# openMVG/openMVG

Hardware: AMD Instinct MI355X
Metric: descriptor pairs/s (brute-force L2 2-NN + ratio matching) (higher is better)
Workload: dtype i8 (int32 accumulate); 1 GPU; 1000 images x 2000 SIFT-like uint8x128 descriptors, exhaustive pairs (499500 image pairs, 499500 on rank 0), ratio 0.8; parallelism=pair-sharded x1, no collective

## Files before the change

openmvg_amd/csrc/mvgx_match.hip:

```cpp
#include <hip/hip_runtime.h>

#include <algorithm>
#include <atomic>
#include <climits>
#include <condition_variable>
#include <cstdint>
#include <cstdlib>
#include <cstring>
#include <functional>
#include <mutex>
#include <string>
#include <thread>
#include <vector>

#include "mvgx_common.h"

namespace {

using mvgx::set_error;

typedef int v4i __attribute__((ext_vector_type(4)));
typedef int v16i __attribute__((ext_vector_type(16)));

constexpr int kDim = 128;
// ... 316 lines not shown
    for (int n = 0; n < kNQ; ++n) { T1[n] = INT_MIN; T2[n] = INT_MIN; }

    const int nt = min(kWinTiles, ntI - win * kWinTiles);
    for (int t = 0; t < nt; ++t) {
      const char* tb = buf + t * kTileBytes + lane * 16;
      v4i a[4];
#pragma unroll
      for (int s = 0; s < 4; ++s) a[s] = *reinterpret_cast<const v4i*>(tb + s * 1024);
      const char* rb = buf + kWinTiles * kTileBytes + t * (kTileRows * 4) + h * 16;
      int R[16];
#pragma unroll
      for (int g = 0; g < 4; ++g) {
        const int4 rv = *reinterpret_cast<const int4*>(rb + g * 32);
        R[g * 4 + 0] = rv.x; R[g * 4 + 1] = rv.y; R[g * 4 + 2] = rv.z; R[g * 4 + 3] = rv.w;
      }
#pragma unroll
      for (int n = 0; n < kNQ; ++n) {
        v16i acc = {0, 0, 0, 0, 0, 0, 0, 0, 0, 0, 0, 0, 0, 0, 0, 0};
#pragma unroll
        for (int s = 0; s < 4; ++s) acc = __builtin_amdgcn_mfma_i32_32x32x32_i8(a[s], b[n][s], acc, 0, 0, 0);
        int t1 = T1[n], t2 = T2[n];
#pragma unroll
        for (int r = 0; r < 16; ++r) {
          const int T = (int)((unsigned)acc[r] << 9) + R[r];
          t2 = med3i(t1, t2, T);
          t1 = max(t1, T);
        }
        T1[n] = t1; T2[n] = t2;
      }
    }
    if constexpr (kMode == kStageRegs) stage_commit(nbuf, sr, wave, lane);
#pragma unroll
    for (int n = 0; n < kNQ; ++n) {
      const int k1 = -T1[n], k2 = -T2[n];
      const int wd1 = k1 >> 8, widx = (k1 & 255) + win * kWinRows, wd2 = k2 >> 8;
      const bool better = wd1 < G1[n];
      const int g2 = better ? min(G1[n], wd2) : min(G2[n], wd1);
      Gi[n] = better ? widx : Gi[n];
      G1[n] = better ? wd1 : G1[n];
      G2[n] = g2;
    }
  }

#pragma unroll
  for (int n = 0; n < kNQ; ++n) {
    const int P1 = __shfl_xor(G1[n], 32), P2 = __shfl_xor(G2[n], 32), Pi = __shfl_xor(Gi[n], 32);
    const bool better = P1 < G1[n];
    const int g2 = better ? min(G1[n], P2) : min(G2[n], P1);
    Gi[n] = better ? Pi : Gi[n];
    G1[n] = better ? P1 : G1[n];
    G2[n] = g2;
  }

#pragma unroll
  for (int n = 0; n < kNQ; ++n) {
    const uint32_t q = (qt0 + n) * kTileRows + (lane & 31);
    const bool inb = (lane < 32) && (qt0 + n < ntJpad);
    bool ok = false;
    if (inb) {
      const bool valid = p.perm[(size_t)tileJ0 * kTileRows + q] != kNoMatch;
      const int nq = p.qnorm[(size_t)tileJ0 * kTileRows + q];
      const int d0 = G1[n] + nq, d1 = G2[n] + nq;
      ok = valid && (__int2float_rn(d0) < __fmul_rn(p.ratio_sq, __int2float_rn(d1)));
      p.best[(size_t)wk.x * p.qstride + q] = ok ? p.perm[(size_t)tileI0 * kTileRows + (uint32_t)Gi[n]] : kNoMatch;
    }
    const unsigned long long m = __ballot(ok);
    if (lane == 0 && m) atomicAdd(&p.count[wk.x], (uint32_t)__popcll(m));
  }
}

__device__ __forceinline__ int max3i(int a, int b, int c) { return max(max(a, b), c); }

template <int kMode, int kDbg = 0>
__global__ __launch_bounds__(256, 2) void l2_filter_kernel(MatchParams p) {
  extern __shared__ __attribute__((aligned(16))) char smem[];

  const int lane = threadIdx.x & 63;
  const int wave = __builtin_amdgcn_readfirstlane(threadIdx.x >> 6);
  const int h = lane >> 5;

  const uint32_t w = xcd_remap(blockIdx.x, gridDim.x);
  const uint2 wk = p.work[w];
  const uint2 ij = p.pairs[wk.x];
  const uint32_t I = ij.x, J = ij.y;
  const uint32_t tileI0 = p.img_tile_off[I], tileJ0 = p.img_tile_off[J];
  const uint32_t ntJpad = p.img_tile_off[J + 1] - tileJ0;
  const int ntI = (int)p.img_ntiles[I];
  const int nwin = (ntI + kWinTiles - 1) / kWinTiles;
  const uint32_t qt0 = wk.y + (uint32_t)wave * kNQ;

  v4i b[kNQ][4];
  {
    const int8_t* qsrc = p.tiles + (size_t)(tileJ0 + qt0) * kTileBytes + lane * 16;
#pragma unroll
    for (int n = 0; n < kNQ; ++n)
#pragma unroll
      for (int s = 0; s < 4; ++s) b[n][s] = *reinterpret_cast<const v4i*>(qsrc + n * kTileBytes + s * 1024);
  }

  const int8_t* gI = p.tiles + (size_t)tileI0 * kTileBytes;
  const int* gC = p.cinit + (size_t)tileI0 * kTileRows;

  constexpr bool kFold = (kDbg & 8) == 0;
  constexpr bool kOneCv = kFold && (kDbg & 16) != 0;
  int TP[kNQ][8];
  int TW[kNQ][8];
  int Q1[kNQ], Q2[kNQ], Qg[kNQ];
#pragma unroll
  for (int n = 0; n < kNQ; ++n) {
#pragma unroll
    for (int s = 0; s < 8; ++s) { TP[n][s] = kNegInit; TW[n][s] = kNegInit; }
    Q1[n] = kNegInit; Q2[n] = kNegInit; Qg[n] = 0;
  }

  StageRegs sr;
  if constexpr (kMode == kStageGlds) {
    stage_window_glds(smem, gI, gC, wave, lane);
  } else if constexpr (kMode == kStageGldsAsm) {
    stage_window_glds_asm(smem, gI, gC, wave, lane);
  } else {
    stage_issue(sr, gI, gC, wave, lane);
    stage_commit(smem, sr, wave, lane);
  }
#pragma unroll
  for (int n = 0; n < kNQ; ++n)
#pragma unroll
    for (int s = 0; s < 4; ++s) asm volatile("" : "+v"(b[n][s]));

  for (int win = 0; win < nwin; ++win) {
    if constexpr (!(kDbg & 4) && kMode == kStageGldsAsm) asm volatile("s_waitcnt vmcnt(0)" ::: "memory");
    if constexpr (!(kDbg & 4)) __syncthreads();
    char* buf = smem + (win & 1) * kStageBytes;
    char* nbuf = smem + ((win + 1) & 1) * kStageBytes;
    if constexpr (kDbg & 4) {
    } else if constexpr (kMode == kStageRegs) {
      const int wn = (win + 1 < nwin) ? win + 1 : win;
      stage_issue(sr, gI + (size_t)wn * kWinTiles * kTileBytes, gC + wn * kWinRows, wave, lane);
    } else if (win + 1 < nwin) {
      const int8_t* gt = gI + (size_t)(win + 1) * kWinTiles * kTileBytes;
      const int* gc = gC + (win + 1) * kWinRows;
      if constexpr (kMode == kStageGlds) stage_window_glds(nbuf, gt, gc, wave, lane);
      else stage_window_glds_asm(nbuf, gt, gc, wave, lane);
    }

    int TQ[kNQ];
#pragma unroll
    for (int n = 0; n < kNQ; ++n) TQ[n] = kNegInit;

    const int nt = min(kWinTiles, ntI - win * kWinTiles);
    const char* wb = buf + lane * 16;
    const char* wc = buf + kWinTiles * kTileBytes + h * 16;
    v4i a[4];
    v16i cv;
#pragma unroll
    for (int s = 0; s < 4; ++s) a[s] = *reinterpret_cast<const v4i*>(wb + s * 1024);
#pragma unroll
    for (int g = 0; g < 4; ++g) {
      const int4 c4 = *reinterpret_cast<const int4*>(wc + g * 32);
      cv[g * 4 + 0] = c4.x; cv[g * 4 + 1] = c4.y; cv[g * 4 + 2] = c4.z; cv[g * 4 + 3] = c4.w;
    }
    v16i accA, accB;
#pragma unroll
    for (int r = 0; r < 16; ++r) accB[r] = kNegInit;

#define MVGX_EPILOGUE(ACC, N)                                          \
  if constexpr (kDbg & 1) { asm volatile("" : "+v"(ACC)); TQ[N] = max(TQ[N], ACC[0]); } else \
  if constexpr (kFold) {                                               \
    _Pragma("unroll") for (int s = 0; s < 8; ++s)                      \
      TW[N][s] = max(max(TW[N][s], ACC[2 * s]), ACC[2 * s + 1]);       \
  } else                                                               \
  {                                                                    \
    int tq = TQ[N];                                                    \
    _Pragma("unroll") for (int s = 0; s < 8; ++s) {                    \
      TP[N][s] = max(max(TP[N][s], ACC[2 * s]), ACC[2 * s + 1]);       \
      tq = max(max(tq, ACC[2 * s + 1]), ACC[2 * s]);                   \
    }                                                                  \
    TQ[N] = tq;                                                        \
  }
#define MVGX_CHAIN(ACC, N, A, CV)                                                            \
  ACC = __builtin_amdgcn_mfma_i32_32x32x32_i8(A[0], b[N][0], CV, 0, 0, 0);                   \
  ACC = __builtin_amdgcn_mfma_i32_32x32x32_i8(A[1], b[N][1], ACC, 0, 0, 0);                  \
  ACC = __builtin_amdgcn_mfma_i32_32x32x32_i8(A[2], b[N][2], ACC, 0, 0, 0);                  \
  ACC = __builtin_amdgcn_mfma_i32_32x32x32_i8(A[3], b[N][3], ACC, 0, 0, 0);
#define MVGX_INTERLEAVE()                                                                    \
  _Pragma("unroll") for (int i_ = 0; i_ < 4; ++i_) {                                         \
    __builtin_amdgcn_sched_group_barrier(0x8, 1, 0);                                         \
    __builtin_amdgcn_sched_group_barrier(0x2, kFold ? 2 : 4, 0);                             \
  }

#define MVGX_TILE(A, CV, AN, CN, TN)                                                              \
  {                                                                                                \
    const int tn_ = (TN);                                                                          \
    MVGX_CHAIN(accA, 0, A, CV)                                                                     \
    if constexpr (kDbg & 2) { _Pragma("unroll") for (int s = 0; s < 4; ++s) AN[s] = A[s]; CN = CV; } else { \
    _Pragma("unroll") for (int s = 0; s < 4; ++s)                                                  \
        AN[s] = *reinterpret_cast<const v4i*>(wb + tn_ * kTileBytes + s * 1024);                   \
    }                                                                                              \
    MVGX_EPILOGUE(accB, 3)                                                                         \
    MVGX_INTERLEAVE()                                                                              \
    MVGX_CHAIN(accB, 1, A, CV)                                                                     \
    if constexpr (!(kDbg & 2) && !kOneCv) {                                                        \
    _Pragma("unroll") for (int g = 0; g < 4; ++g) {                                                \
      const int4 c4 = *reinterpret_cast<const int4*>(wc + tn_ * (kTileRows * 4) + g * 32);        \
      CN[g * 4 + 0] = c4.x; CN[g * 4 + 1] = c4.y; CN[g * 4 + 2] = c4.z; CN[g * 4 + 3] = c4.w;     \
    }                                                                                              \
    }                                                                                              \
    MVGX_EPILOGUE(accA, 0)                                                                         \
    MVGX_INTERLEAVE()                                                                              \
    MVGX_CHAIN(accA, 2, A, CV)                                                                     \
    MVGX_EPILOGUE(accB, 1)                                                                         \
    MVGX_INTERLEAVE()                                                                              \
    if constexpr (kOneCv) {   \
      accB = __builtin_amdgcn_mfma_i32_32x32x32_i8(A[0], b[3][0], CV, 0, 0, 0);                   \
      if constexpr (!(kDbg & 2))                                                                   \
      _Pragma("unroll") for (int g = 0; g < 4; ++g) {                                              \
        const int4 c4 = *reinterpret_cast<const int4*>(wc + tn_ * (kTileRows * 4) + g * 32);      \
        CV[g * 4 + 0] = c4.x; CV[g * 4 + 1] = c4.y; CV[g * 4 + 2] = c4.z; CV[g * 4 + 3] = c4.w;   \
      }                                                                                            \
      accB = __builtin_amdgcn_mfma_i32_32x32x32_i8(A[1], b[3][1], accB, 0, 0, 0);                 \
      accB = __builtin_amdgcn_mfma_i32_32x32x32_i8(A[2], b[3][2], accB, 0, 0, 0);                 \
      accB = __builtin_amdgcn_mfma_i32_32x32x32_i8(A[3], b[3][3], accB, 0, 0, 0);                 \
    } else {                                                                                       \
      MVGX_CHAIN(accB, 3, A, CV)                                                                   \
    }                                                                                              \
    MVGX_EPILOGUE(accA, 2)                                                                         \
    MVGX_INTERLEAVE()                                                                              \
  }
    v4i an[4];
    v16i cn;
    int t = 0;
    if constexpr (kOneCv) {
      for (; t + 1 < nt; t += 2) {
        MVGX_TILE(a, cv, an, cv, t + 1)
        MVGX_TILE(an, cv, a, cv, min(t + 2, nt - 1))
      }
      if (t < nt) MVGX_TILE(a, cv, an, cv, t)
    } else {
      for (; t + 1 < nt; t += 2) {
        MVGX_TILE(a, cv, an, cn, t + 1)
        MVGX_TILE(an, cn, a, cv, min(t + 2, nt - 1))
      }
      if (t < nt) MVGX_TILE(a, cv, an, cn, t)
    }
    MVGX_EPILOGUE(accB, 3)
#undef MVGX_EPILOGUE
#undef MVGX_CHAIN
#undef MVGX_TILE
#undef MVGX_INTERLEAVE
    if constexpr (kMode == kStageRegs) stage_commit(nbuf, sr, wave, lane);
    if constexpr (kFold) {
#pragma unroll
      for (int n = 0; n < kNQ; ++n) {
        int tq = max(max(TW[n][0], TW[n][1]), TW[n][2]);
        tq = max(max(tq, TW[n][3]), TW[n][4]);
        tq = max(max(tq, TW[n][5]), TW[n][6]);
        TQ[n] = max(tq, TW[n][7]);
#pragma unroll
        for (int s = 0; s < 8; ++s) { TP[n][s] = max(TP[n][s], TW[n][s]); TW[n][s] = kNegInit; }
      }
    }
#pragma unroll
    for (int n = 0; n < kNQ; ++n) {
      const int v = TQ[n];
      const bool better = v > Q1[n];
      Q2[n] = better ? Q1[n] : max(Q2[n], v);
      Qg[n] = better ? win : Qg[n];
      Q1[n] = better ? v : Q1[n];
    }
  }

#pragma unroll
  for (int n = 0; n < kNQ; ++n) {
    int p1 = kNegInit, p2 = kNegInit, ps = 0;
#pragma unroll
    for (int s = 0; s < 8; ++s) {
      const int v = TP[n][s];
      const bool better = v > p1;
      p2 = better ? p1 : max(p2, v);
      ps = better ? s : ps;
      p1 = better ? v : p1;
    }
    const int w1 = 2 * p1 - h, w2p = 2 * p2 - h, w2q = 2 * Q2[n] - h;
    const int o1 = __shfl_xor(w1, 32), o2p = __shfl_xor(w2p, 32), o2q = __shfl_xor(w2q, 32);
    const int os = __shfl_xor(ps, 32), og = __shfl_xor(Qg[n], 32);
    const bool mine = w1 > o1;
    const int W1 = mine ? w1 : o1;
    const int V2 = mine ? max3i(w2p, w2q, o1) : max3i(o2p, o2q, w1);
    const int s1 = mine ? ps : os, g1 = mine ? Qg[n] : og, hw = mine ? h : (h ^ 1);

    const uint32_t q = (qt0 + n) * kTileRows + (lane & 31);
    if (lane < 32 && qt0 + n < ntJpad) {
      const bool valid = p.perm[(size_t)tileJ0 * kTileRows + q] != kNoMatch;
      const int nq = p.qnorm[(size_t)tileJ0 * kTileRows + q];
      const int d0 = nq - W1, d1ub = nq - V2;
      const bool cand = valid && (__int2float_rn(d0) < __fmul_rn(p.ratio_sq, __int2float_rn(d1ub)));
      const size_t o = (size_t)wk.x * p.qstride + q;
      p.best[o] = cand ? ((uint32_t)s1 | ((uint32_t)hw << 3) | ((uint32_t)g1 << 4)) : kNoMatch;
      if (cand) p.cd[o] = make_int2(d0, d1ub);
    }
  }
}

constexpr int kNB16 = 2 * kNQ;
__global__ __launch_bounds__(256, 2) void l2_filter16_kernel(MatchParams p) {
  extern __shared__ __attribute__((aligned(16))) char smem[];

  const int lane = threadIdx.x & 63;
  const int wave = __builtin_amdgcn_readfirstlane(threadIdx.x >> 6);
  const int g4 = lane >> 4, par = g4 & 1;

  const uint32_t w = xcd_remap(blockIdx.x, gridDim.x);
  const uint4* rec = p.work8 + (size_t)kRecQuads * w;
  const uint4 wsh = rec[0], wun = rec[1 + wave];
  const uint32_t tileI0 = wsh.x;
  const int ntI = (int)wsh.y;
  const uint32_t pair = wun.x, tileJ0 = wun.y, qt0 = wun.z;
  const uint32_t nJ = wun.w;
  const int nwin = (ntI + kWinTiles - 1) / kWinTiles;

  const int lane_chunk = ((lane >> 5) * 64 + ((lane >> 4) & 1) * 32 + (lane & 15)) * 16;
  v4i b[kNB16][2];
  {
    const int8_t* qsrc = p.qtiles + (size_t)(tileJ0 + qt0) * kTileBytes + lane_chunk;
#pragma unroll
    for (int n = 0; n < kNB16; ++n)
#pragma unroll
      for (int ks = 0; ks < 2; ++ks) b[n][ks] = *reinterpret_cast<const v4i*>(qsrc + (n >> 1) * kTileBytes + (n & 1) * 256 + ks * 2048);
  }

  const int8_t* gI = p.tiles + (size_t)tileI0 * kTileBytes;
  const int* gC = p.cinit + (size_t)tileI0 * kTileRows;

  int qn[kNB16];
#pragma unroll
  for (int n = 0; n < kNB16; ++n) {
    const uint32_t q = (qt0 + (uint32_t)(n >> 1)) * kTileRows + (uint32_t)(n & 1) * 16 + (uint32_t)(lane & 15);
    qn[n] = (lane < 16 && q < nJ) ? p.qtnorm[(size_t)tileJ0 * kTileRows + q] : 0;
  }

  int TP[kNB16][4];
  int TW[kNB16][4];
  int Q1[kNB16], Q2[kNB16], Qg[kNB16];
#pragma unroll
  for (int n = 0; n < kNB16; ++n) {
#pragma unroll
    for (int c = 0; c < 4; ++c) { TP[n][c] = kNegInit; TW[n][c] = kNegInit; }
    Q1[n] = kNegInit; Q2[n] = kNegInit; Qg[n] = 0;
  }

  stage_window_glds_asm(smem, gI, gC, wave, lane);
#pragma unroll
  for (int n = 0; n < kNB16; ++n) {
#pragma unroll
    for (int ks = 0; ks < 2; ++ks) asm volatile("" : "+v"(b[n][ks]));
    asm volatile("" : "+v"(qn[n]));
  }

  for (int win = 0; win < nwin; ++win) {
    asm volatile("s_waitcnt vmcnt(0)" ::: "memory");
    __syncthreads();
    char* buf = smem + (win & 1) * kStageBytes;
    char* nbuf = smem + ((win + 1) & 1) * kStageBytes;
    if (win + 1 < nwin)
      stage_window_glds_asm(nbuf, gI + (size_t)(win + 1) * kWinTiles * kTileBytes, gC + (win + 1) * kWinRows, wave, lane);

    const int nt = min(kWinTiles, ntI - win * kWinTiles);
    const char* wb = buf + lane_chunk;
    const char* wc = buf + kWinTiles * kTileBytes + g4 * 16;
    v4i accA[4], accB[4];
#pragma unroll
    for (int i = 0; i < 4; ++i) accB[i] = v4i{kNegInit, kNegInit, kNegInit, kNegInit};

#define MVGX_GROUP16(ACC, N0, A, CV)                                                                       \
  _Pragma("unroll") for (int i_ = 0; i_ < 4; ++i_)                                                          \
    ACC[i_] = __builtin_amdgcn_mfma_i32_16x16x64_i8(A[0], b[(N0) + i_][0], CV, 0, 0, 0);                    \
  _Pragma("unroll") for (int i_ = 0; i_ < 4; ++i_)                                                          \
    ACC[i_] = __builtin_amdgcn_mfma_i32_16x16x64_i8(A[1], b[(N0) + i_][1], ACC[i_], 0, 0, 0);
#define MVGX_EPI16(ACC, N0, BLK)                                                                            \
  _Pragma("unroll") for (int i_ = 0; i_ < 4; ++i_) {                                                        \
    TW[(N0) + i_][2 * (BLK)] = max(max(TW[(N0) + i_][2 * (BLK)], ACC[i_][0]), ACC[i_][1]);                  \
    TW[(N0) + i_][2 * (BLK) + 1] = max(max(TW[(N0) + i_][2 * (BLK) + 1], ACC[i_][2]), ACC[i_][3]);          \
  }
#define MVGX_MIX16(NDS)                                                                                     \
  _Pragma("unroll") for (int i_ = 0; i_ < 8; ++i_) {                                                        \
    __builtin_amdgcn_sched_group_barrier(0x8, 1, 0);                                                        \
    __builtin_amdgcn_sched_group_barrier(0x2, 1, 0);                                                        \
    if (i_ < (NDS)) __builtin_amdgcn_sched_group_barrier(0x100, 1, 0);                                      \
  }
#define MVGX_BLOCK16(A, CV, AN, CN, BLK, NEXT_OFF, NEXT_COFF)                                               \
  {                                                                                                         \
    MVGX_GROUP16(accA, 0, A, CV)                                                                            \
    AN[0] = *reinterpret_cast<const v4i*>(wb + (NEXT_OFF));                                                 \
    AN[1] = *reinterpret_cast<const v4i*>(wb + (NEXT_OFF) + 2048);                                          \
    MVGX_EPI16(accB, 4, 1 - (BLK))                                                                          \
    MVGX_MIX16(2)                                                                                           \
    MVGX_GROUP16(accB, 4, A, CV)                                                                            \
    CN = *reinterpret_cast<const v4i*>(wc + (NEXT_COFF));                                                   \
    MVGX_EPI16(accA, 0, BLK)                                                                                \
    MVGX_MIX16(1)                                                                                           \
  }
    v4i a0[2], a1[2], c0, c1;
    a0[0] = *reinterpret_cast<const v4i*>(wb);
    a0[1] = *reinterpret_cast<const v4i*>(wb + 2048);
    c0 = *reinterpret_cast<const v4i*>(wc);
    __builtin_amdgcn_s_setprio(3);
    for (int t = 0; t < nt; ++t) {
      const int tn = min(t + 1, nt - 1);
      MVGX_BLOCK16(a0, c0, a1, c1, 0, t * kTileBytes + 256, t * (kTileRows * 4) + 64)
      MVGX_BLOCK16(a1, c1, a0, c0, 1, tn * kTileBytes, tn * (kTileRows * 4))
    }
    MVGX_EPI16(accB, 4, 1)
    __builtin_amdgcn_s_setprio(0);
#undef MVGX_GROUP16
#undef MVGX_EPI16
#undef MVGX_MIX16
#undef MVGX_BLOCK16
#pragma unroll
    for (int n = 0; n < kNB16; ++n) {
      const int v = max(max(max(TW[n][0], TW[n][1]), TW[n][2]), TW[n][3]);
#pragma unroll
      for (int c = 0; c < 4; ++c) { TP[n][c] = max(TP[n][c], TW[n][c]); TW[n][c] = kNegInit; }
      const bool better = v > Q1[n];
      Q2[n] = better ? Q1[n] : max(Q2[n], v);
      Qg[n] = better ? win : Qg[n];
      Q1[n] = better ? v : Q1[n];
    }
  }

#pragma unroll
  for (int n = 0; n < kNB16; ++n) {
    int p1 = kNegInit, p2 = kNegInit, pc = 0;
#pragma unroll
    for (int c = 0; c < 4; ++c) {
      const int v = TP[n][c];
      const bool better = v > p1;
      p2 = better ? p1 : max(p2, v);
      pc = better ? c : pc;
      p1 = better ? v : p1;
    }
    int W1 = 2 * p1 - par, V2 = max(2 * p2 - par, 2 * Q2[n] - par);
    int code = (4 * (pc >> 1) + 2 * (g4 >> 1) + (pc & 1)) | (par << 3) | (Qg[n] << 4);
#pragma unroll
    for (int x = 16; x <= 32; x <<= 1) {
      const int o1 = __shfl_xor(W1, x), o2 = __shfl_xor(V2, x), oc = __shfl_xor(code, x);
      const bool mine = W1 > o1;
      V2 = mine ? max(V2, o1) : max(o2, W1);
      code = mine ? code : oc;
      W1 = mine ? W1 : o1;
    }
    const uint32_t q = (qt0 + (uint32_t)(n >> 1)) * kTileRows + (uint32_t)(n & 1) * 16 + (uint32_t)(lane & 15);
    if (lane < 16 && q < nJ) {
      const int nq = qn[n];
      const int d0 = nq - W1, d1ub = nq - V2;
      const bool cand = __int2float_rn(d0) < __fmul_rn(p.ratio_sq, __int2float_rn(d1ub));
      const size_t o = (size_t)pair * p.qstride + q;
      p.best[o] = cand ? (uint32_t)code : kNoMatch;
      if (cand) p.cd[o] = make_int2(d0, d1ub);
    }
  }
}

constexpr int kNQh = 2;
constexpr int kNBh = 2 * kNQh;
constexpr int kBlockQTilesH = kWaves * kNQh;
__global__ __launch_bounds__(256, 3) void l2_filter16h_kernel(MatchParams p) {
  extern __shared__ __attribute__((aligned(16))) char smem[];

  const int lane = threadIdx.x & 63;
  const int wave = __builtin_amdgcn_readfirstlane(threadIdx.x >> 6);
  const int g4 = lane >> 4, par = g4 & 1;

  const uint32_t w = xcd_remap(blockIdx.x, gridDim.x);
  const uint4 wr0 = p.work8h[2 * (size_t)w], wr1 = p.work8h[2 * (size_t)w + 1];
  const uint32_t pair = wr0.x;
  const uint32_t tileI0 = wr0.z, tileJ0 = wr0.w;
  const uint32_t ntJpad = wr1.y;
  const int ntI = (int)wr1.x;
  const int nhalf = (ntI + kHalfTiles - 1) / kHalfTiles;
  const uint32_t qt0 = wr0.y + (uint32_t)wave * kNQh;

  const int lane_chunk = ((lane >> 5) * 64 + ((lane >> 4) & 1) * 32 + (lane & 15)) * 16;
  v4i b[kNBh][2];
  {
    const int8_t* qsrc = p.tiles + (size_t)(tileJ0 + qt0) * kTileBytes + lane_chunk;
#pragma unroll
    for (int n = 0; n < kNBh; ++n)
#pragma unroll
      for (int ks = 0; ks < 2; ++ks) b[n][ks] = *reinterpret_cast<const v4i*>(qsrc + (n >> 1) * kTileBytes + (n & 1) * 256 + ks * 2048);
  }
  const int8_t* gI = p.tiles + (size_t)tileI0 * kTileBytes;
  const int* gC = p.cinit + (size_t)tileI0 * kTileRows;

  uint32_t qperm[kNBh];
  int qn[kNBh];
#pragma unroll
  for (int n = 0; n < kNBh; ++n) {
    const bool inb = lane < 16 && qt0 + (uint32_t)(n >> 1) < ntJpad;
    const size_t qs = (size_t)tileJ0 * kTileRows + (qt0 + (uint32_t)(n >> 1)) * kTileRows + (uint32_t)(n & 1) * 16 + (uint32_t)(lane & 15);
    qperm[n] = inb ? p.perm[qs] : kNoMatch;
    qn[n] = inb ? p.qnorm[qs] : 0;
  }

  int TP[kNBh][4], TW[kNBh][4], Q1[kNBh], Q2[kNBh], Qg[kNBh];
#pragma unroll
  for (int n = 0; n < kNBh; ++n) {
#pragma unroll
    for (int c = 0; c < 4; ++c) { TP[n][c] = kNegInit; TW[n][c] = kNegInit; }
    Q1[n] = kNegInit; Q2[n] = kNegInit; Qg[n] = 0;
  }

  stage_half_glds_asm(smem, gI, gC, wave, lane);
#pragma unroll
  for (int n = 0; n < kNBh; ++n) {
#pragma unroll
    for (int ks = 0; ks < 2; ++ks) asm volatile("" : "+v"(b[n][ks]));
    asm volatile("" : "+v"(qperm[n]), "+v"(qn[n]));
  }

  for (int hw = 0; hw < nhalf; ++hw) {
    asm volatile("s_waitcnt vmcnt(0)" ::: "memory");
    __syncthreads();
    char* buf = smem + (hw & 1) * kHalfStageBytes;
    char* nbuf = smem + ((hw + 1) & 1) * kHalfStageBytes;
    if (hw + 1 < nhalf)
      stage_half_glds_asm(nbuf, gI + (size_t)(hw + 1) * kHalfTiles * kTileBytes, gC + (hw + 1) * kHalfTiles * kTileRows, wave, lane);

    const int nt = min(kHalfTiles, ntI - hw * kHalfTiles);
    const char* wb = buf + lane_chunk;
    const char* wc = buf + kHalfTiles * kTileBytes + g4 * 16;
    v4i accA[4], accB[4];
#pragma unroll
    for (int i = 0; i < 4; ++i) accB[i] = v4i{kNegInit, kNegInit, kNegInit, kNegInit};
#define MVGX_GROUPH(ACC, A, CV)                                                                              \
  _Pragma("unroll") for (int i_ = 0; i_ < 4; ++i_)                                                          \
    ACC[i_] = __builtin_amdgcn_mfma_i32_16x16x64_i8(A[0], b[i_][0], CV, 0, 0, 0);                           \
  _Pragma("unroll") for (int i_ = 0; i_ < 4; ++i_)                                                          \
    ACC[i_] = __builtin_amdgcn_mfma_i32_16x16x64_i8(A[1], b[i_][1], ACC[i_], 0, 0, 0);
#define MVGX_EPIH(ACC, BLK)                                                                                  \
  _Pragma("unroll") for (int i_ = 0; i_ < 4; ++i_) {                                                        \
    TW[i_][2 * (BLK)] = max(max(TW[i_][2 * (BLK)], ACC[i_][0]), ACC[i_][1]);                                \
    TW[i_][2 * (BLK) + 1] = max(max(TW[i_][2 * (BLK) + 1], ACC[i_][2]), ACC[i_][3]);                        \
  }
#define MVGX_MIXH(NDS)                                                                                       \
  _Pragma("unroll") for (int i_ = 0; i_ < 8; ++i_) {                                                        \
    __builtin_amdgcn_sched_group_barrier(0x8, 1, 0);                                                        \
    __builtin_amdgcn_sched_group_barrier(0x2, 1, 0);                                                        \
    if (i_ < (NDS)) __builtin_amdgcn_sched_group_barrier(0x100, 1, 0);                                      \
  }
    v4i a0[2], a1[2], c0, c1;
    a0[0] = *reinterpret_cast<const v4i*>(wb);
    a0[1] = *reinterpret_cast<const v4i*>(wb + 2048);
    c0 = *reinterpret_cast<const v4i*>(wc);
    for (int t = 0; t < nt; ++t) {
      const int tn = min(t + 1, nt - 1);
      MVGX_GROUPH(accA, a0, c0)
      a1[0] = *reinterpret_cast<const v4i*>(wb + t * kTileBytes + 256);
      a1[1] = *reinterpret_cast<const v4i*>(wb + t * kTileBytes + 256 + 2048);
      c1 = *reinterpret_cast<const v4i*>(wc + t * (kTileRows * 4) + 64);
      MVGX_EPIH(accB, 1)
      MVGX_MIXH(3)
      MVGX_GROUPH(accB, a1, c1)
      a0[0] = *reinterpret_cast<const v4i*>(wb + tn * kTileBytes);
      a0[1] = *reinterpret_cast<const v4i*>(wb + tn * kTileBytes + 2048);
      c0 = *reinterpret_cast<const v4i*>(wc + tn * (kTileRows * 4));
      MVGX_EPIH(accA, 0)
      MVGX_MIXH(3)
    }
    MVGX_EPIH(accB, 1)
#undef MVGX_GROUPH
#undef MVGX_EPIH
#undef MVGX_MIXH
    if ((hw & 1) || hw + 1 == nhalf) {
      const int win = hw >> 1;
#pragma unroll
      for (int n = 0; n < kNBh; ++n) {
        const int v = max(max(max(TW[n][0], TW[n][1]), TW[n][2]), TW[n][3]);
#pragma unroll
        for (int c = 0; c < 4; ++c) { TP[n][c] = max(TP[n][c], TW[n][c]); TW[n][c] = kNegInit; }
        const bool better = v > Q1[n];
        Q2[n] = better ? Q1[n] : max(Q2[n], v);
        Qg[n] = better ? win : Qg[n];
        Q1[n] = better ? v : Q1[n];
      }
    }
  }

#pragma unroll
  for (int n = 0; n < kNBh; ++n) {
    int p1 = kNegInit, p2 = kNegInit, pc = 0;
#pragma unroll
    for (int c = 0; c < 4; ++c) {
      const int v = TP[n][c];
      const bool better = v > p1;
      p2 = better ? p1 : max(p2, v);
      pc = better ? c : pc;
      p1 = better ? v : p1;
    }
    int W1 = 2 * p1 - par, V2 = max(2 * p2 - par, 2 * Q2[n] - par);
    int code = (4 * (pc >> 1) + 2 * (g4 >> 1) + (pc & 1)) | (par << 3) | (Qg[n] << 4);
#pragma unroll
    for (int x = 16; x <= 32; x <<= 1) {
      const int o1 = __shfl_xor(W1, x), o2 = __shfl_xor(V2, x), oc = __shfl_xor(code, x);
      const bool mine = W1 > o1;
      V2 = mine ? max(V2, o1) : max(o2, W1);
      code = mine ? code : oc;
      W1 = mine ? W1 : o1;
    }
    const uint32_t q = (qt0 + (uint32_t)(n >> 1)) * kTileRows + (uint32_t)(n & 1) * 16 + (uint32_t)(lane & 15);
    if (lane < 16 && qt0 + (uint32_t)(n >> 1) < ntJpad) {
      const bool valid = qperm[n] != kNoMatch;
      const int nq = qn[n];
      const int d0 = nq - W1, d1ub = nq - V2;
      const bool cand = valid && (__int2float_rn(d0) < __fmul_rn(p.ratio_sq, __int2float_rn(d1ub)));
      const size_t o = (size_t)pair * p.qstride + q;
      p.best[o] = cand ? (uint32_t)code : kNoMatch;
      if (cand) p.cd[o] = make_int2(d0, d1ub);
    }
  }
}

template <bool kWaveUnits>
__global__ __launch_bounds__(256) void l2_verify_kernel(MatchParams p) {
  const int lane = threadIdx.x & 63;
  const int wave = threadIdx.x >> 6;
  uint32_t pair, qt0, I, tileI0, tileJ0, qend;
  const uint8_t* rowsJ = nullptr;
  if constexpr (kWaveUnits) {
    const uint4* rec = p.work8 + (size_t)kRecQuads * blockIdx.x;
    const uint4 wun = rec[1 + __builtin_amdgcn_readfirstlane(wave)];
    pair = wun.x; tileJ0 = wun.y; qt0 = wun.z; qend = wun.w;
    tileI0 = rec[0].x;
    const uint2 ij = p.pairs[pair];
    I = ij.x;
    rowsJ = p.rows_u8 + p.img_row_off[ij.y] * kDim;
  } else {
    const uint2 wk = p.work[blockIdx.x];
    const uint2 ij = p.pairs[wk.x];
    pair = wk.x; qt0 = wk.y + (uint32_t)wave * kNQ;
    I = ij.x;
    tileI0 = p.img_tile_off[I]; tileJ0 = p.img_tile_off[ij.y];
    qend = (p.img_tile_off[ij.y + 1] - tileJ0) * kTileRows;
  }
  const uint32_t nEvenI = p.img_neven[I], nOddI = p.img_n[I] - nEvenI;
  const int l16 = lane & 15, sub = lane >> 4;
  uint32_t accepted = 0;
  for (int part = 0; part < 2; ++part) {
    const uint32_t q0 = qt0 * kTileRows + (uint32_t)part * 64;
    const uint32_t q = q0 + lane;
    const bool inb = q < qend;
    const uint32_t code = inb ? p.best[(size_t)pair * p.qstride + q] : kNoMatch;
    unsigned long long todo = __ballot(code != kNoMatch);
    while (todo) {
      unsigned long long m = todo;
      for (int i = 0; i < sub; ++i) m &= m - 1;
      const bool active = m != 0;
      const int src = active ? __builtin_ctzll(m) : 0;
      for (int i = 0; i < 4; ++i) todo &= todo - 1;
      const uint32_t cc = (uint32_t)__shfl((int)code, src);
      const uint32_t qs = q0 + (uint32_t)src;
      const int s1 = cc & 7, hw = (cc >> 3) & 1, g1 = (int)(cc >> 4);
      const int piece = l16 & 7, rsel = l16 >> 3;
      const int mrow = slot_row(2 * s1 + rsel, hw);
      const size_t slot0 = (size_t)tileI0 * kTileRows + (active ? (size_t)g1 * kWinTiles * kTileRows + mrow : 0);
      const size_t slotQ = (size_t)tileJ0 * kTileRows + (active ? qs : 0);
      const size_t o = (size_t)pair * p.qstride + (active ? qs : 0);
      const uint32_t tt = (uint32_t)g1 * kWinTiles + (uint32_t)piece;
      const size_t slotI = active ? slot0 + (size_t)piece * kTileRows : slot0;
      const bool valid = active && (tt * 16u + (uint32_t)(2 * s1 + rsel)) < (hw ? nOddI : nEvenI);
      int4 va[8];
#pragma unroll
      for (int c = 0; c < 8; ++c)
        va[c] = *reinterpret_cast<const int4*>(p.rows_slot + (slot0 + (active ? (size_t)c * kTileRows : 0)) * kDim + piece * 16);
      int4 vb;
      if constexpr (kWaveUnits) {
        vb = *reinterpret_cast<const int4*>(rowsJ + (size_t)(active ? qs : 0) * kDim + piece * 16);
        vb.x ^= (int)0x80808080u; vb.y ^= (int)0x80808080u; vb.z ^= (int)0x80808080u; vb.w ^= (int)0x80808080u;
      } else {
        vb = *reinterpret_cast<const int4*>(p.rows_slot + slotQ * kDim + piece * 16);
      }
      const int2 f = p.cd[o];
      const int f_d0 = f.x, f_d1 = f.y;
      int nb = __builtin_amdgcn_sdot4(vb.x, vb.x, 0, false);
      nb = __builtin_amdgcn_sdot4(vb.y, vb.y, nb, false);
      nb = __builtin_amdgcn_sdot4(vb.z, vb.z, nb, false);
      nb = __builtin_amdgcn_sdot4(vb.w, vb.w, nb, false);
      nb += __builtin_amdgcn_update_dpp(0, nb, 0xB1, 0xF, 0xF, true);
      nb += __builtin_amdgcn_update_dpp(0, nb, 0x4E, 0xF, 0xF, true);
      nb += __builtin_amdgcn_update_dpp(0, nb, 0x141, 0xF, 0xF, true);
      int dot = 0, na = 0;
#pragma unroll
      for (int c = 0; c < 8; ++c) {
        int part = __builtin_amdgcn_sdot4(va[c].x, vb.x, 0, false);
        part = __builtin_amdgcn_sdot4(va[c].y, vb.y, part, false);
        part = __builtin_amdgcn_sdot4(va[c].z, vb.z, part, false);
        part = __builtin_amdgcn_sdot4(va[c].w, vb.w, part, false);
        part += __builtin_amdgcn_update_dpp(0, part, 0xB1, 0xF, 0xF, true);
        part += __builtin_amdgcn_update_dpp(0, part, 0x4E, 0xF, 0xF, true);
        part += __builtin_amdgcn_update_dpp(0, part, 0x141, 0xF, 0xF, true);
        dot = (c == piece) ? part : dot;
        int sq = __builtin_amdgcn_sdot4(va[c].x, va[c].x, 0, false);
        sq = __builtin_amdgcn_sdot4(va[c].y, va[c].y, sq, false);
        sq = __builtin_amdgcn_sdot4(va[c].z, va[c].z, sq, false);
        sq = __builtin_amdgcn_sdot4(va[c].w, va[c].w, sq, false);
        sq += __builtin_amdgcn_update_dpp(0, sq, 0xB1, 0xF, 0xF, true);
        sq += __builtin_amdgcn_update_dpp(0, sq, 0x4E, 0xF, 0xF, true);
        sq += __builtin_amdgcn_update_dpp(0, sq, 0x141, 0xF, 0xF, true);
        na = (c == piece) ? sq : na;
      }
      const int d = valid ? na + nb - 2 * dot : INT_MAX;
      int key = valid ? ((d << 4) | l16) : INT_MAX;
      key = min(key, __builtin_amdgcn_update_dpp(INT_MAX, key, 0xB1, 0xF, 0xF, false));
      key = min(key, __builtin_amdgcn_update_dpp(INT_MAX, key, 0x4E, 0xF, 0xF, false));
      key = min(key, __builtin_amdgcn_update_dpp(INT_MAX, key, 0x141, 0xF, 0xF, false));
      key = min(key, __builtin_amdgcn_update_dpp(INT_MAX, key, 0x140, 0xF, 0xF, false));
      const int wl = key & 15, dbest = key >> 4;
      int second = (l16 == wl) ? INT_MAX : d;
      second = min(second, __builtin_amdgcn_update_dpp(INT_MAX, second, 0xB1, 0xF, 0xF, false));
      second = min(second, __builtin_amdgcn_update_dpp(INT_MAX, second, 0x4E, 0xF, 0xF, false));
      second = min(second, __builtin_amdgcn_update_dpp(INT_MAX, second, 0x141, 0xF, 0xF, false));
      second = min(second, __builtin_amdgcn_update_dpp(INT_MAX, second, 0x140, 0xF, 0xF, false));
      bool ok = false;
      if (active && l16 == wl) {
        if (key == INT_MAX || dbest != f_d0) atomicAdd(p.errflag, 1u);
        const int d1 = min(f_d1, second);
        ok = __int2float_rn(dbest) < __fmul_rn(p.ratio_sq, __int2float_rn(d1));
        p.best[o] = ok ? p.perm[slotI] : kNoMatch;
      }
      accepted += (uint32_t)__popcll(__ballot(ok));
    }
  }
  if (lane == 0 && accepted) atomicAdd(&p.count[pair], accepted);
}

__global__ __launch_bounds__(256) void count_candidates_kernel(const uint32_t* __restrict__ best, size_t n,
                                                               uint32_t* __restrict__ counter) {
  __shared__ uint32_t s_sum;
  if (threadIdx.x == 0) s_sum = 0;
  __syncthreads();
  uint32_t c = 0;
  const size_t base = (size_t)blockIdx.x * 16384;
  for (int k = 0; k < 64; ++k) {
    const size_t i = base + (size_t)k * 256 + threadIdx.x;
    if (i < n && best[i] != kNoMatch) ++c;
  }
  const unsigned long long m = __ballot(c != 0);
  (void)m;
  for (int off = 32; off > 0; off >>= 1) c += __shfl_down(c, off);
  if ((threadIdx.x & 63) == 0 && c) atomicAdd(&s_sum, c);
  __syncthreads();
  if (threadIdx.x == 0 && s_sum) atomicAdd(counter, s_sum);
}

__global__ __launch_bounds__(256) void count_candidates_units_kernel(MatchParams p, uint32_t* __restrict__ counter) {
  __shared__ uint32_t s_sum;
  if (threadIdx.x == 0) s_sum = 0;
  __syncthreads();
  const int lane = threadIdx.x & 63, wave = threadIdx.x >> 6;
  const uint4 wun = p.work8[(size_t)kRecQuads * blockIdx.x + 1 + wave];
  uint32_t c = 0;
  for (int part = 0; part < 2; ++part) {
    const uint32_t q = wun.z * kTileRows + (uint32_t)part * 64 + (uint32_t)lane;
    const bool cand = q < wun.w && p.best[(size_t)wun.x * p.qstride + q] != kNoMatch;
// ... 667 lines not shown
        hipLaunchKernelGGL(l2_filter_kernel<kStageGlds>, dim3(n_work), dim3(256), 2 * kStageBytes, stream, mp);
      } else if (c->debug_filter) {
#define MVGX_DBG_CASE(D) case D: hipLaunchKernelGGL((l2_filter_kernel<kStageGldsAsm, D>), dim3(n_work), dim3(256), 2 * kStageBytes, stream, mp); break;
        switch (c->debug_filter) {
#ifdef MVGX_FILTER_TIMING_VARIANTS
          MVGX_DBG_CASE(1) MVGX_DBG_CASE(2) MVGX_DBG_CASE(3) MVGX_DBG_CASE(4) MVGX_DBG_CASE(5) MVGX_DBG_CASE(6) MVGX_DBG_CASE(7)
#endif
          MVGX_DBG_CASE(8) MVGX_DBG_CASE(16) default: break; }
#undef MVGX_DBG_CASE
      } else {
        hipLaunchKernelGGL(l2_filter_kernel<kStageGldsAsm>, dim3(n_work), dim3(256), 2 * kStageBytes, stream, mp);
      }
      MVGX_HIP(hipGetLastError());
      if (c->profile) MVGX_HIP(hipEventRecord(e1, stream));
      if (!c->verify_alone) MVGX_HIP(hipEventRecord(sl.ev_filter, stream));
      st.n_kernel_launches += 1;
      if (c->variant == 4 && !(c->debug_filter & 7)) {
        if (c->profile >= 2) {
          const size_t nslots = (size_t)nb * c->qstride;
          if (records)
            hipLaunchKernelGGL(count_candidates_units_kernel, dim3(n_rec), dim3(256), 0, stream, mp, c->d_err.p + 1);
          else
            hipLaunchKernelGGL(count_candidates_kernel, dim3((unsigned)((nslots + 16383) / 16384)), dim3(256), 0, stream,
                               sl.d_best.p, nslots, c->d_err.p + 1);
        }
        if (records)
          hipLaunchKernelGGL(l2_verify_kernel<true>, dim3(n_rec), dim3(256), 0, stream, mp);
        else
          hipLaunchKernelGGL(l2_verify_kernel<false>, dim3(n_work), dim3(256), 0, stream, mp);
        MVGX_HIP(hipGetLastError());
      }
      if (c->verify_alone) MVGX_HIP(hipEventRecord(sl.ev_filter, stream));
    }
    if (!n_work) MVGX_HIP(hipEventRecord(sl.ev_filter, stream));
    hipLaunchKernelGGL(scan_counts_kernel, dim3(1), dim3(1024), 0, stream, sl.d_count.p, nb, sl.d_offsets.p);
    MVGX_HIP(hipGetLastError());
    MVGX_HIP(hipMemcpyAsync(sl.hp_offsets.p, sl.d_offsets.p, ((size_t)nb + 1) * sizeof(uint32_t), hipMemcpyDeviceToHost, stream));
    MVGX_HIP(hipEventRecord(sl.ev_scan, stream));
    return MVGX_OK;
  };
  auto finish = [&](mvgx_match_ctx::Slot& sl) -> int {
    int rc;
    MVGX_HIP(hipEventSynchronize(sl.ev_scan));
    const uint32_t nb = sl.nb;
    const uint64_t p0 = sl.p0;
    const uint32_t total = sl.hp_offsets.p[nb];
    if (sink) {
      if (c->stream_hold) sl.out_set ^= 1;
      sl.h_off_out[sl.out_set].assign(sl.hp_offsets.p, sl.hp_offsets.p + nb + 1);
    } else {
      const uint64_t base = res.offsets[p0];
      for (uint32_t k = 0; k <= nb; ++k) res.offsets[p0 + k] = base + sl.hp_offsets.p[k];
    }
    sl.out_p0 = p0; sl.out_nb = nb;
    st.n_matches += total;
    if (total) {
      if ((rc = sl.d_ij.ensure(total))) return rc;
      hipLaunchKernelGGL(compact_matches_kernel, dim3((nb + 3) / 4), dim3(256), 0, sl.stream, sl.d_best.p,
                         sl.d_offsets.p, sl.d_pairs.p, c->d_n.p, c->d_row_off.p, dense_queries ? nullptr : c->d_rowpos.p, nb, c->qstride,
                         sl.d_ij.p);
      MVGX_HIP(hipGetLastError());
      if (sink) {
        PinnedBuf<uint32_t>& hb = sl.hp_ij[sl.out_set];
        if (!hb.p) hb.pageable = !c->pinned_stream;
        if ((size_t)total * 2 > hb.cap) { hb.release(); if ((rc = hb.grow_keep(std::max<size_t>((size_t)total * 3, 4u << 20), 0))) return rc; }
        MVGX_HIP(hipMemcpyAsync(hb.p, sl.d_ij.p, (size_t)total * sizeof(uint2), hipMemcpyDeviceToHost, sl.stream));
      } else if (c->keep_host_results) {
        const size_t old = res.ij_n;
        if (old + (size_t)total * 2 > res.ij.cap)
          for (auto& o : c->slot) MVGX_HIP(hipStreamSynchronize(o.stream));
        if ((rc = res.ij.grow_keep(old + (size_t)total * 2, old))) return rc;
        res.ij_n = old + (size_t)total * 2;
        MVGX_HIP(hipMemcpyAsync(res.ij.p + old, sl.d_ij.p, (size_t)total * sizeof(uint2),
                                hipMemcpyDeviceToHost, sl.stream));
      }
    }
    if (sink) MVGX_HIP(hipEventRecord(sl.ev_copy, sl.stream));
    return MVGX_OK;
  };
  auto deliver = [&](mvgx_match_ctx::Slot& sl) -> int {
    MVGX_HIP(hipEventSynchronize(sl.ev_copy));
    if (feed.stop.load()) return MVGX_OK;
    if ((*sink)(sl.out_p0, sl.out_nb, sl.h_off_out[sl.out_set].data(), sl.hp_ij[sl.out_set].p)) feed.stop.store(1);
    return MVGX_OK;
  };
  uint64_t nbatch = 0, p0 = 0;
  uint32_t nb = 0;
  while (feed.take(p0, nb)) {
    mvgx_match_ctx::Slot& cur = c->slot[nbatch & 1];
    mvgx_match_ctx::Slot* prev = nbatch ? &c->slot[(nbatch - 1) & 1] : nullptr;
    if (!c->overlap) {
      if ((rc = issue(cur, nullptr, p0, nb)) || (rc = finish(cur))) return rc;
      MVGX_HIP(hipStreamSynchronize(cur.stream));
      if (sink && (rc = deliver(cur))) return rc;
      ++nbatch;
      continue;
    }
    if ((rc = issue(cur, prev, p0, nb))) return rc;
    if (prev && (rc = finish(*prev))) return rc;
    if (sink && nbatch >= 2 && (rc = deliver(cur))) return rc;
    ++nbatch;
  }
  if (c->overlap && nbatch) {
    mvgx_match_ctx::Slot& last = c->slot[(nbatch - 1) & 1];
    if (sink && nbatch >= 2 && (rc = deliver(c->slot[nbatch & 1]))) return rc;
    if ((rc = finish(last))) return rc;
    if (sink && (rc = deliver(last))) return rc;
  }
  for (auto& sl : c->slot) MVGX_HIP(hipStreamSynchronize(sl.stream));
  MVGX_HIP(hipEventRecord(c->ev_total1, c->slot[0].stream));
  MVGX_HIP(hipEventSynchronize(c->ev_total1));
  float ms = 0.f;
  MVGX_HIP(hipEventElapsedTime(&ms, c->ev_total0, c->ev_total1));
  st.total_ms = ms;
  if (c->variant == 4 && !(c->debug_filter & 7)) {
    uint32_t flags[2] = {0, 0};
    MVGX_HIP(hipMemcpy(flags, c->d_err.p, 2 * sizeof(uint32_t), hipMemcpyDeviceToHost));
    (void)hipMemset(c->d_err.p, 0, 2 * sizeof(uint32_t));
    const uint32_t nerr = flags[0];
    st.kernel_vgprs = flags[1];
    if (nerr) {
      set_error("matching filter/verify disagreement on %u candidates (internal error)", nerr);
      return MVGX_ERR_NUMERIC;
    }
  }
  if (c->profile) {
    for (size_t i = 0; i + 1 < n_ev; i += 2) {
      float k = 0.f;
      MVGX_HIP(hipEventElapsedTime(&k, c->ev_pool[i], c->ev_pool[i + 1]));
      st.kernel_ms += k;
    }
  }
  return MVGX_OK;
}

void add_stats(mvgx_match_stats& a, const mvgx_match_stats& b) {
  a.n_pairs += b.n_pairs; a.n_desc_pairs += b.n_desc_pairs; a.n_matches += b.n_matches;
  a.n_kernel_launches += b.n_kernel_launches; a.kernel_ms += b.kernel_ms;
  a.total_ms = std::max(a.total_ms, b.total_ms); a.kernel_vgprs += b.kernel_vgprs; a.variant = b.variant;
}

int run_multi(mvgx_match_ctx* c, BatchFeed& feed, float ratio_sq, const BatchSink& sink, mvgx_match_stats& st) {
  const size_t nd = c->children.size();
  struct Mail { uint64_t p0; uint32_t nb; const uint32_t* offsets; const uint32_t* ij; int result; bool full, done; };
  std::mutex mu;
  std::condition_variable cv_main, cv_dev;
  std::vector<Mail> mail(nd, Mail{0, 0, nullptr, nullptr, 0, false, false});
  std::vector<int> rcs(nd, MVGX_OK);
  std::vector<std::string> errs(nd);
  std::vector<mvgx_match_stats> sts(nd);
  size_t running = nd;
  std::vector<std::thread> workers;
  for (size_t d = 0; d < nd; ++d) {
    workers.emplace_back([&, d]() {
      BatchSink post = [&, d](uint64_t p0, uint32_t nb, const uint32_t* offsets, const uint32_t* ij) -> int {
        std::unique_lock<std::mutex> lk(mu);
        mail[d] = Mail{p0, nb, offsets, ij, 0, true, false};
        cv_main.notify_one();
        cv_dev.wait(lk, [&]() { return mail[d].done; });
        mail[d].full = mail[d].done = false;
        return mail[d].result;
      };
      rcs[d] = run_device(c->children[d], feed, ratio_sq, &post, sts[d]);
      if (rcs[d] != MVGX_OK) { errs[d] = mvgx_last_error(); feed.stop.store(1); }
      std::lock_guard<std::mutex> lk(mu);
      --running;
      cv_main.notify_one();
    });
  }
  {
    std::unique_lock<std::mutex> lk(mu);
    for (;;) {
      size_t ready = nd;
      cv_main.wait(lk, [&]() {
        for (size_t d = 0; d < nd; ++d)
          if (mail[d].full && !mail[d].done) { ready = d; return true; }
        return running == 0;
      });
      if (ready == nd) break;
      Mail m = mail[ready];
      if (feed.stop.load()) {
        mail[ready].result = 1;
        mail[ready].done = true;
        cv_dev.notify_all();
        continue;
      }
      lk.unlock();
      const int r = sink(m.p0, m.nb, m.offsets, m.ij);
      if (r != 0) feed.stop.store(1);
      lk.lock();
      mail[ready].result = r;
      mail[ready].done = true;
      cv_dev.notify_all();
    }
  }
  for (auto& w : workers) w.join();
  memset(&st, 0, sizeof(st));
  int rc = MVGX_OK;
  for (size_t d = 0; d < nd; ++d) {
    add_stats(st, sts[d]);
    if (rcs[d] != MVGX_OK && rc == MVGX_OK) { rc = rcs[d]; set_error("device %d: %s", c->children[d]->device, errs[d].c_str()); }
  }
  return rc;
}

int check_run_args(mvgx_match_ctx* c, const uint32_t* pairs_IJ, uint64_t n_pairs, float ratio_sq, const char* who) {
  MVGX_REQUIRE(c && (pairs_IJ || n_pairs == 0), MVGX_ERR_ARG, "%s: NULL argument", who);
  const mvgx_match_ctx* r = c->children.empty() ? c : c->children[0];
  MVGX_REQUIRE(r->d_rows_view != nullptr || r->n_images == 0, MVGX_ERR_STATE, "%s before set_regions", who);
  MVGX_REQUIRE(ratio_sq <= 1.0f && ratio_sq >= 0.0f, MVGX_ERR_UNSUPPORTED,
               "ratio_sq = %g: the device path reproduces the reference only for 0 <= ratio^2 <= 1 "
               "(ties are libstdc++ partial_sort order beyond that)", (double)ratio_sq);
  for (uint64_t k = 0; k < n_pairs; ++k)
    MVGX_REQUIRE(pairs_IJ[2 * k] < r->n_images && pairs_IJ[2 * k + 1] < r->n_images, MVGX_ERR_ARG,
                 "pair %llu references image out of range", (unsigned long long)k);
  return MVGX_OK;
}

uint64_t batch_size(const mvgx_match_ctx* c) {
  const mvgx_match_ctx* r = c->children.empty() ? c : c->children[0];
  return std::max<uint64_t>(1, std::min<uint64_t>((uint64_t)c->batch_pairs, std::max<uint64_t>(16, (1ull << 29) / std::max<uint32_t>(r->qstride, 1))));
}

}

extern "C" {

int mvgx_match_run(mvgx_match_ctx* c, const uint32_t* pairs_IJ, uint64_t n_pairs, float ratio_sq,
                   mvgx_match_stats* stats) {
  int rc = check_run_args(c, pairs_IJ, n_pairs, ratio_sq, "mvgx_match_run");
  if (rc) return rc;
  if (c->double_buffer) c->cur ^= 1;
  mvgx_match_ctx::Results& res = c->results[c->cur];
  res.offsets.assign(n_pairs + 1, 0);
  res.ij_n = 0;
  BatchFeed feed;
  feed.pairs_IJ = pairs_IJ; feed.n_pairs = n_pairs; feed.B = batch_size(c);
  mvgx_match_stats st;
  if (c->children.empty()) {
    rc = run_device(c, feed, ratio_sq, nullptr, st);
  } else {
    struct Piece { uint64_t p0; std::vector<uint32_t> ij; };
    std::vector<Piece> pieces;
    BatchSink collect = [&](uint64_t p0, uint32_t nb, const uint32_t* offsets, const uint32_t* ij) -> int {
      for (uint32_t k = 0; k < nb; ++k) res.offsets[p0 + k + 1] = offsets[k + 1] - offsets[k];
      if (c->keep_host_results && offsets[nb]) pieces.push_back(Piece{p0, std::vector<uint32_t>(ij, ij + 2 * (size_t)offsets[nb])});
      return 0;
    };
    rc = run_multi(c, feed, ratio_sq, collect, st);
    if (rc == MVGX_OK) {
      for (uint64_t k = 0; k < n_pairs; ++k) res.offsets[k + 1] += res.offsets[k];
      if (c->keep_host_results) {
        if ((rc = res.ij.grow_keep(2 * res.offsets[n_pairs], 0))) return rc;
        res.ij_n = 2 * res.offsets[n_pairs];
        for (const Piece& p : pieces) memcpy(res.ij.p + 2 * res.offsets[p.p0], p.ij.data(), p.ij.size() * sizeof(uint32_t));
      }
    }
  }
  if (rc == MVGX_OK && stats) *stats = st;
  return rc;
}

int mvgx_match_run_stream(mvgx_match_ctx* c, const uint32_t* pairs_IJ, uint64_t n_pairs, float ratio_sq,
                          mvgx_match_batch_sink sink, void* user, mvgx_match_stats* stats) {
  int rc = check_run_args(c, pairs_IJ, n_pairs, ratio_sq, "mvgx_match_run_stream");
  if (rc) return rc;
  MVGX_REQUIRE(sink != nullptr, MVGX_ERR_ARG, "mvgx_match_run_stream: sink is NULL");
  BatchFeed feed;
  feed.pairs_IJ = pairs_IJ; feed.n_pairs = n_pairs; feed.B = batch_size(c);
  BatchSink fn = [&](uint64_t p0, uint32_t nb, const uint32_t* offsets, const uint32_t* ij) -> int {
    return sink(user, p0, nb, offsets, ij);
  };
  mvgx_match_stats st;
  rc = c->children.empty() ? run_device(c, feed, ratio_sq, &fn, st) : run_multi(c, feed, ratio_sq, fn, st);
  if (rc == MVGX_OK && stats) *stats = st;
  return rc;
}

int mvgx_match_results(mvgx_match_ctx* c, const uint64_t** offsets, const uint32_t** ij) {
  MVGX_REQUIRE(c && offsets && ij, MVGX_ERR_ARG, "mvgx_match_results: NULL argument");
  *offsets = c->results[c->cur].offsets.data();
  *ij = c->results[c->cur].ij.p;
  return MVGX_OK;
}

int mvgx_match_pairs_u8_l2(const uint8_t* const* desc_rows, const uint32_t* n_desc, uint32_t n_images,
                           uint32_t dim, const uint32_t* pairs_IJ, uint64_t n_pairs, float ratio_sq, int device,
                           mvgx_match_sink sink, void* user) {
  mvgx_match_ctx* c = nullptr;
  int rc = mvgx_match_create(device, &c);
  if (rc) return rc;
  rc = mvgx_match_set_regions(c, desc_rows, n_desc, n_images, dim);
  if (!rc) rc = mvgx_match_run(c, pairs_IJ, n_pairs, ratio_sq, nullptr);
  if (!rc && sink) {
    for (uint64_t k = 0; k < n_pairs; ++k) {
      const uint64_t a = c->results[c->cur].offsets[k], b = c->results[c->cur].offsets[k + 1];
      if (b > a) sink(user, pairs_IJ[2 * k], pairs_IJ[2 * k + 1], c->results[c->cur].ij.p + 2 * a, (uint32_t)(b - a));
    }
  }
  mvgx_match_destroy(c);
  return rc;
}

}
```

Measured before the change: 10300 billion descriptor pairs/s.

## Interleave next-window staging into the MFMA tile loop of l2_filter16

Instead of issuing the whole next-window global-to-LDS stage at the top of each window, the kernel now issues one tile piece per inner-loop iteration (plus the row-constant piece on the first iteration), spreading load traffic across the compute loop. The wait and barrier move to the end of the window, and the next window's first fragments are preloaded right after that barrier. It also adds compile-time-gated timestamp instrumentation and a host readout function, both disabled by default. The intent is smoother overlap of staging with MFMA work. The risk is that the extra per-iteration branches and issue slots disturb the tuned instruction schedule.

```diff
diff --git a/openmvg_amd/csrc/mvgx_match.hip b/openmvg_amd/csrc/mvgx_match.hip
--- a/openmvg_amd/csrc/mvgx_match.hip
+++ b/openmvg_amd/csrc/mvgx_match.hip
@@ -642,12 +642,49 @@
 }
 
 constexpr int kNB16 = 2 * kNQ;
+
+#ifdef MVGX_FILTER_EDGE_STAMPS
+constexpr uint32_t kStampWgs = 4096, kStampEvery = 8;
+__device__ unsigned g_edge_stamps[kStampWgs][kWaves][64];
+#define MVGX_STAMP(SLOT)                                                             \
+  {                                                                                  \
+    __builtin_amdgcn_sched_barrier(0);                                               \
+    const unsigned t_ = (unsigned)__builtin_amdgcn_s_memtime();                      \
+    if (lane == 0) stamp_lds[wave][(SLOT)] = t_ - stamp_t0;                          \
+    __builtin_amdgcn_sched_barrier(0);                                               \
+  }
+#define MVGX_STAMP_TOP(WIN, K, FIRST) { if ((WIN) == 0) { if (FIRST) MVGX_STAMP(FIRST) } else if ((WIN) < 12) MVGX_STAMP(5 * (WIN) + (K)) }
+#define MVGX_STAMP_END(WIN, K) { if ((WIN) + 1 < 12) MVGX_STAMP(5 * ((WIN) + 1) + (K)) }
+#else
+#define MVGX_STAMP(SLOT)
+#define MVGX_STAMP_TOP(WIN, K, FIRST)
+#define MVGX_STAMP_END(WIN, K)
+#endif
+__device__ __forceinline__ void stage_piece(char* buf, const int8_t* __restrict__ gtiles, const int* __restrict__ grconst, int i, int wave, int lane) {
+  const int off = i * kTileBytes + wave * (i < kWinTiles ? 1024 : 256);
+#if defined(__HIP_DEVICE_COMPILE__)
+  const unsigned lds = __builtin_amdgcn_readfirstlane((unsigned)(size_t)(__attribute__((address_space(3))) char*)buf + off);
+  if (i < kWinTiles) glds16_asm(gtiles + off + lane * 16, lds);
+  else glds4_asm(grconst + wave * 64 + lane, lds);
+#else
+  if (i < kWinTiles) memcpy(buf + off + lane * 16, gtiles + off + lane * 16, 16);
+  else memcpy(buf + off + lane * 4, grconst + wave * 64 + lane, 4);
+#endif
+}
+constexpr int kEdgePieces = 1;
 __global__ __launch_bounds__(256, 2) void l2_filter16_kernel(MatchParams p) {
   extern __shared__ __attribute__((aligned(16))) char smem[];
 
   const int lane = threadIdx.x & 63;
   const int wave = __builtin_amdgcn_readfirstlane(threadIdx.x >> 6);
   const int g4 = lane >> 4, par = g4 & 1;
+#ifdef MVGX_FILTER_EDGE_STAMPS
+  __shared__ unsigned stamp_lds[kWaves][64];
+  stamp_lds[wave][lane] = 0;
+  const unsigned stamp_t0 = (unsigned)__builtin_amdgcn_s_memtime();
+  const unsigned stamp_r0 = (unsigned)__builtin_amdgcn_s_memrealtime();
+  if (lane == 0) stamp_lds[wave][0] = stamp_t0;
+#endif
 
   const uint32_t w = xcd_remap(blockIdx.x, gridDim.x);
   const uint4* rec = p.work8 + (size_t)kRecQuads * w;
@@ -657,6 +694,10 @@
   const uint32_t pair = wun.x, tileJ0 = wun.y, qt0 = wun.z;
   const uint32_t nJ = wun.w;
   const int nwin = (ntI + kWinTiles - 1) / kWinTiles;
+#ifdef MVGX_FILTER_EDGE_STAMPS
+  asm volatile("" ::"s"(ntI), "s"(qt0), "s"(nJ));
+#endif
+  MVGX_STAMP(1)
 
   const int lane_chunk = ((lane >> 5) * 64 + ((lane >> 4) & 1) * 32 + (lane & 15)) * 16;
   v4i b[kNB16][2];
@@ -695,14 +736,22 @@
     for (int ks = 0; ks < 2; ++ks) asm volatile("" : "+v"(b[n][ks]));
     asm volatile("" : "+v"(qn[n]));
   }
+  MVGX_STAMP(2)
+
+  asm volatile("s_waitcnt vmcnt(0)" ::: "memory");
+  MVGX_STAMP(3)
+  __syncthreads();
+  v4i a0[2], a1[2], c0, c1;
+  a0[0] = *reinterpret_cast<const v4i*>(smem + lane_chunk);
+  a0[1] = *reinterpret_cast<const v4i*>(smem + lane_chunk + 2048);
+  c0 = *reinterpret_cast<const v4i*>(smem + kWinTiles * kTileBytes + g4 * 16);
 
   for (int win = 0; win < nwin; ++win) {
-    asm volatile("s_waitcnt vmcnt(0)" ::: "memory");
-    __syncthreads();
     char* buf = smem + (win & 1) * kStageBytes;
     char* nbuf = smem + ((win + 1) & 1) * kStageBytes;
-    if (win + 1 < nwin)
-      stage_window_glds_asm(nbuf, gI + (size_t)(win + 1) * kWinTiles * kTileBytes, gC + (win + 1) * kWinRows, wave, lane);
+    const bool stage_next = win + 1 < nwin;
+    const int8_t* gnt = gI + (size_t)(win + 1) * kWinTiles * kTileBytes;
+    const int* gnc = gC + (win + 1) * kWinRows;
 
     const int nt = min(kWinTiles, ntI - win * kWinTiles);
     const char* wb = buf + lane_chunk;
@@ -739,18 +788,30 @@
     MVGX_EPI16(accA, 0, BLK)                                                                                \
     MVGX_MIX16(1)                                                                                           \
   }
-    v4i a0[2], a1[2], c0, c1;
-    a0[0] = *reinterpret_cast<const v4i*>(wb);
-    a0[1] = *reinterpret_cast<const v4i*>(wb + 2048);
-    c0 = *reinterpret_cast<const v4i*>(wc);
+    MVGX_STAMP_TOP(win, 3, 4)
     __builtin_amdgcn_s_setprio(3);
     for (int t = 0; t < nt; ++t) {
       const int tn = min(t + 1, nt - 1);
+      if (stage_next && t < kWinTiles / kEdgePieces) {
+#pragma unroll
+        for (int k = 0; k < kEdgePieces; ++k) stage_piece(nbuf, gnt, gnc, t * kEdgePieces + k, wave, lane);
+        if (t == 0) stage_piece(nbuf, gnt, gnc, kWinTiles, wave, lane);
+      }
       MVGX_BLOCK16(a0, c0, a1, c1, 0, t * kTileBytes + 256, t * (kTileRows * 4) + 64)
       MVGX_BLOCK16(a1, c1, a0, c0, 1, tn * kTileBytes, tn * (kTileRows * 4))
     }
     MVGX_EPI16(accB, 4, 1)
     __builtin_amdgcn_s_setprio(0);
+    MVGX_STAMP_END(win, 0)
+    if (stage_next) {
+      asm volatile("s_waitcnt vmcnt(0)" ::: "memory");
+      MVGX_STAMP_END(win, 1)
+      __syncthreads();
+      MVGX_STAMP_END(win, 2)
+      a0[0] = *reinterpret_cast<const v4i*>(nbuf + lane_chunk);
+      a0[1] = *reinterpret_cast<const v4i*>(nbuf + lane_chunk + 2048);
+      c0 = *reinterpret_cast<const v4i*>(nbuf + kWinTiles * kTileBytes + g4 * 16);
+    }
 #undef MVGX_GROUP16
 #undef MVGX_EPI16
 #undef MVGX_MIX16
@@ -765,7 +826,9 @@
       Qg[n] = better ? win : Qg[n];
       Q1[n] = better ? v : Q1[n];
     }
-  }
+    MVGX_STAMP_END(win, 4)
+  }
+  MVGX_STAMP(60)
 
 #pragma unroll
   for (int n = 0; n < kNB16; ++n) {
@@ -798,6 +861,14 @@
       if (cand) p.cd[o] = make_int2(d0, d1ub);
     }
   }
+#ifdef MVGX_FILTER_EDGE_STAMPS
+  MVGX_STAMP(61)
+  if (lane == 0) {
+    stamp_lds[wave][62] = (unsigned)__builtin_amdgcn_s_memrealtime() - stamp_r0;
+    stamp_lds[wave][63] = (unsigned)__builtin_amdgcn_s_memtime() - stamp_t0;
+  }
+  if (w % kStampEvery == 0 && w / kStampEvery < kStampWgs) g_edge_stamps[w / kStampEvery][wave][lane] = stamp_lds[wave][lane];
+#endif
 }
 
 constexpr int kNQh = 2;
@@ -2071,4 +2142,12 @@
   return rc;
 }
 
-}
+#ifdef MVGX_FILTER_EDGE_STAMPS
+int mvgx_match_edge_stamps(uint32_t* out, uint64_t words) {
+  MVGX_REQUIRE(out && words == (uint64_t)kStampWgs * kWaves * 64, MVGX_ERR_ARG, "mvgx_match_edge_stamps: 4096 x 4 x 64 words");
+  MVGX_HIP(hipDeviceSynchronize());
+  MVGX_HIP(hipMemcpyFromSymbol(out, HIP_SYMBOL(g_edge_stamps), words * sizeof(uint32_t)));
+  return MVGX_OK;
+}
+#endif
+}
```

Result: no change. 10380 billion descriptor pairs/s, median of 6 (+0.8%).
